# Exidekat/TransformerUpscaler

Measured on AMD Instinct MI355X. Metric: images/sec, FastTransformer 2x 720p->1080p inference, higher is better.
Workload: dtype bf16

## Files before the change

### transformerupscaler_amd/csrc/common.h

```cpp
#pragma once
#include <hip/hip_runtime.h>
#include <stdint.h>
#include <stdlib.h>
#include "tupscale_hip.h"

#ifdef TUP_DIAG
extern "C" {
int tup_debug_tail_stamps(unsigned long long* host_out);
int tup_debug_bs_stamps(unsigned long long* host_out);
int tup_debug_block32_stamps(unsigned long long* host_out);
int tup_debug_conv_stamps(unsigned long long* host_out);
}
#endif

typedef __bf16 bf16_t;
typedef __attribute__((ext_vector_type(8))) __bf16 bf16x8;
typedef __attribute__((ext_vector_type(4))) __bf16 bf16x4;
typedef __attribute__((ext_vector_type(2))) __bf16 bf16x2;
typedef __attribute__((ext_vector_type(4))) short s16x4;
typedef __attribute__((ext_vector_type(4))) float f32x4;
typedef __attribute__((ext_vector_type(4))) uint32_t u32x4;
typedef __attribute__((ext_vector_type(2))) uint32_t u32x2;

#define TUP_DEVICE __device__ __forceinline__

TUP_DEVICE uint32_t lds_addr(const void* p) {
    return (uint32_t)(uintptr_t)(const __attribute__((address_space(3))) char*)(p);
}
TUP_DEVICE bf16x8 lds_read_b128_asm(uint32_t addr) {
    bf16x8 v;
    asm volatile("ds_read_b128 %0, %1" : "=v"(v) : "v"(addr));
    return v;
}
TUP_DEVICE bf16x8 lds_read_b128_asm_off(uint32_t addr, int off) {
    bf16x8 v;
    asm volatile("ds_read_b128 %0, %1 offset:%2" : "=v"(v) : "v"(addr), "i"(off));
    return v;
}
TUP_DEVICE bf16x8 lds_read_b128_asm_off_x64(uint32_t addr, int off) {
    bf16x8 v;
    uint32_t tmp;
    asm volatile("v_xor_b32 %1, 64, %2\n\tds_read_b128 %0, %1 offset:%3" : "=v"(v), "=&v"(tmp) : "v"(addr), "i"(off));
    return v;
}
template <int N> TUP_DEVICE void lds_wait() { asm volatile("s_waitcnt lgkmcnt(%0)" ::"n"(N) : "memory"); }

TUP_DEVICE float bf16_to_f32(bf16_t v) { return static_cast<float>(v); }
TUP_DEVICE bf16_t f32_to_bf16(float v) { return static_cast<bf16_t>(v); }

TUP_DEVICE uint32_t pack_bf16x2(float lo, float hi) {
    bf16x2 p = {static_cast<bf16_t>(lo), static_cast<bf16_t>(hi)};
    return __builtin_bit_cast(uint32_t, p);
}

TUP_DEVICE f32x4 mfma16x16x32(bf16x8 a, bf16x8 b, f32x4 c) {
    return __builtin_amdgcn_mfma_f32_16x16x32_bf16(a, b, c, 0, 0, 0);
}
TUP_DEVICE f32x4 mfma16x16x16(s16x4 a, s16x4 b, f32x4 c) {
    return __builtin_amdgcn_mfma_f32_16x16x16bf16_1k(a, b, c, 0, 0, 0);
}

TUP_DEVICE int swz128(int row, int chunk) { return row * 128 + ((chunk ^ ((row >> 1) & 7)) << 4); }

TUP_DEVICE int lane_id_fresh() {
    int l;
    asm volatile("v_mbcnt_lo_u32_b32 %0, -1, 0\n\tv_mbcnt_hi_u32_b32 %0, -1, %0" : "=v"(l));
    return l;
}
TUP_DEVICE uint32_t opaque_copy(uint32_t u) { asm volatile("" : "+v"(u)); return u; }
TUP_DEVICE float vmax(float a, float b) { float r; asm("v_max_f32 %0, %1, %2" : "=v"(r) : "v"(a), "v"(b)); return r; }
TUP_DEVICE float rows_max(float v) {
    const uint32_t u = __builtin_bit_cast(uint32_t, v);
    const auto r = __builtin_amdgcn_permlane16_swap(u, u, false, false);
    const float m = vmax(__builtin_bit_cast(float, r[0]), __builtin_bit_cast(float, opaque_copy(r[1])));
    const uint32_t w = __builtin_bit_cast(uint32_t, m);
    const auto q = __builtin_amdgcn_permlane32_swap(w, w, false, false);
    return vmax(__builtin_bit_cast(float, q[0]), __builtin_bit_cast(float, opaque_copy(q[1])));
}
TUP_DEVICE float rows_sum(float v) {
    const uint32_t u = __builtin_bit_cast(uint32_t, v);
    const auto r = __builtin_amdgcn_permlane16_swap(u, u, false, false);
    const float m = __builtin_bit_cast(float, r[0]) + __builtin_bit_cast(float, opaque_copy(r[1]));
    const uint32_t w = __builtin_bit_cast(uint32_t, m);
    const auto q = __builtin_amdgcn_permlane32_swap(w, w, false, false);
    return __builtin_bit_cast(float, q[0]) + __builtin_bit_cast(float, opaque_copy(q[1]));
}

typedef __attribute__((ext_vector_type(2))) float f32x2;

TUP_DEVICE f32x2 fast_erf2(f32x2 z) {
    f32x2 zc;
    zc[0] = fminf(fmaxf(z[0], -2.9f), 2.9f);
    zc[1] = fminf(fmaxf(z[1], -2.9f), 2.9f);
    const f32x2 w = zc * zc;
    f32x2 q = w * 1.2033207800518448e-08f + -4.4140491617154536e-07f;
    q = q * w + 6.2528506609435753e-06f;
    q = q * w + -3.6053944566514376e-05f;
    q = q * w + -7.2369640518118916e-05f;
    q = q * w + 0.0026871317284937087f;
    q = q * w + -0.02176163837525465f;
    q = q * w + 0.10692235311582286f;
    q = q * w + -0.37271276562605715f;
    q = q * w + 1.1276929106383919f;
    return zc * q;
}
TUP_DEVICE float fast_erf(float z) { return fast_erf2(f32x2{z, z})[0]; }

template <int N>
TUP_DEVICE void gelu_erf2_batch(f32x2 (&x)[N]) {
    f32x2 xc[N], u[N], q[N];
#pragma unroll
    for (int i = 0; i < N; ++i) {
        xc[i][0] = __builtin_amdgcn_fmed3f(x[i][0], -4.16f, 4.16f);
        xc[i][1] = __builtin_amdgcn_fmed3f(x[i][1], -4.16f, 4.16f);
        u[i] = xc[i] * xc[i];
        q[i] = u[i] * -9.3762207218685175e-10f + 8.1762115989189489e-08f;
    }
    constexpr float C[6] = {-3.0998062963740323e-06f, 6.7728779820009944e-05f, -0.00095683661677124407f, 0.0093223106686782069f,
                            -0.065572048515984249f, 0.39849236879961203f};
#pragma unroll
    for (int k = 0; k < 6; ++k)
#pragma unroll
        for (int i = 0; i < N; ++i) q[i] = q[i] * u[i] + C[k];
#pragma unroll
    for (int i = 0; i < N; ++i) x[i] = x[i] * (xc[i] * q[i] + 0.5f);
}

typedef _Float16 h2 __attribute__((ext_vector_type(2)));
typedef _Float16 h8 __attribute__((ext_vector_type(8)));
template <int N>
TUP_DEVICE void gelu16_batch(h2 (&x)[N]) {
    const h2 one = {(_Float16)1.0f, (_Float16)1.0f};
    h2 xc[N], sv[N], q[N];
#pragma unroll
    for (int i = 0; i < N; ++i) {
        xc[i] = __builtin_elementwise_min(__builtin_elementwise_max(x[i], -one), one);
        sv[i] = __builtin_elementwise_fma(xc[i], xc[i], h2{(_Float16)-0.5f, (_Float16)-0.5f});
        q[i] = __builtin_elementwise_fma(sv[i], h2{(_Float16)1.51615563f, (_Float16)1.51615563f}, h2{(_Float16)-2.11659751f, (_Float16)-2.11659751f});
    }
    constexpr float C[5] = {1.54543088f, -1.13520344f, 0.88632128f, -0.6753973f, 0.70388307f};
#pragma unroll
    for (int k = 0; k < 5; ++k)
#pragma unroll
        for (int i = 0; i < N; ++i) q[i] = __builtin_elementwise_fma(q[i], sv[i], h2{(_Float16)C[k], (_Float16)C[k]});
#pragma unroll
    for (int i = 0; i < N; ++i) x[i] = x[i] * __builtin_elementwise_fma(xc[i], q[i], h2{(_Float16)0.5f, (_Float16)0.5f});
}
template <int TGN>
TUP_DEVICE void gelu16_fragments(const f32x4 (&acc1)[TGN][2], bf16x8 (&hfr)[TGN]) {
    h2 hv[4 * TGN];
#pragma unroll
    for (int tg = 0; tg < TGN; ++tg)
#pragma unroll
        for (int hh = 0; hh < 2; ++hh) {
            hv[tg * 4 + hh * 2 + 0] = __builtin_convertvector(f32x2{acc1[tg][hh][0], acc1[tg][hh][1]}, h2);
            hv[tg * 4 + hh * 2 + 1] = __builtin_convertvector(f32x2{acc1[tg][hh][2], acc1[tg][hh][3]}, h2);
        }
#ifndef TUP_EXP_NOGELU
    gelu16_batch<4 * TGN>(hv);
#endif
#pragma unroll
    for (int tg = 0; tg < TGN; ++tg) {
        u32x4 pk;
#pragma unroll
        for (int q = 0; q < 4; ++q) pk[q] = __builtin_bit_cast(uint32_t, hv[tg * 4 + q]);
        hfr[tg] = __builtin_bit_cast(bf16x8, pk);
    }
}
TUP_DEVICE f32x4 mfma16x16x32_f16(bf16x8 a, bf16x8 b, f32x4 c) {
    return __builtin_amdgcn_mfma_f32_16x16x32_f16(__builtin_bit_cast(h8, a), __builtin_bit_cast(h8, b), c, 0, 0, 0);
}

TUP_DEVICE f32x2 gelu_erf2(f32x2 x) {
    f32x2 v[1] = {x};
    gelu_erf2_batch<1>(v);
    return v[0];
}
TUP_DEVICE float gelu_erf(float x) { return gelu_erf2(f32x2{x, x})[0]; }

TUP_DEVICE float gelu_erf_grad(float x) {
    return 0.5f * (1.0f + fast_erf(x * 0.70710678118654752440f)) + x * 0.39894228040143267794f * __expf(-0.5f * x * x);
}

TUP_DEVICE uint32_t drop_hash(uint32_t seed, uint32_t idx) {
#ifdef TUP_CHEAP_HASH
    return idx * 0x9E3779B1u + seed;
#endif
    uint32_t h = idx * 0x9E3779B1u + seed;
    h ^= h >> 16; h *= 0x85EBCA6Bu; h ^= h >> 13; h *= 0xC2B2AE35u; h ^= h >> 16;
    return h;
}
TUP_DEVICE float drop_scale(uint32_t seed, uint32_t idx, uint32_t thresh, float inv_keep) {
    return drop_hash(seed, idx) >= thresh ? inv_keep : 0.f;
}
TUP_DEVICE float drop_pair_lo(uint32_t h, uint32_t thresh_hi, float inv_keep) { return (h << 16) >= thresh_hi ? inv_keep : 0.f; }
TUP_DEVICE float drop_pair_hi(uint32_t h, uint32_t thresh_hi, float inv_keep) { return h >= thresh_hi ? inv_keep : 0.f; }
TUP_DEVICE float drop_pair(uint32_t seed, uint32_t idx, uint32_t thresh_hi, float inv_keep) {
    const uint32_t h = drop_hash(seed, idx >> 1);
    return ((idx & 1u) ? h : (h << 16)) >= thresh_hi ? inv_keep : 0.f;
}
TUP_DEVICE void drop_pair4(uint32_t seed, uint32_t idx0, uint32_t thresh_hi, float inv_keep, float (&m)[4]) {
    const uint32_t h0 = drop_hash(seed, idx0 >> 1), h1 = drop_hash(seed, (idx0 >> 1) + 1u);
    m[0] = drop_pair_lo(h0, thresh_hi, inv_keep); m[1] = drop_pair_hi(h0, thresh_hi, inv_keep);
    m[2] = drop_pair_lo(h1, thresh_hi, inv_keep); m[3] = drop_pair_hi(h1, thresh_hi, inv_keep);
}
TUP_DEVICE void drop_pair4_rows(uint32_t seed, uint32_t idx0, uint32_t ncols, uint32_t thresh_hi, float inv_keep, float (&m)[4]) {
    const bool odd = (idx0 & 1u) != 0u;
    const uint32_t ia = (idx0 + (odd ? 2u * ncols : 0u)) >> 1;
    const uint32_t ha = drop_hash(seed, ia), hb = drop_hash(seed, ia + (ncols >> 1));
    const uint32_t pa = (uint32_t)__builtin_amdgcn_update_dpp(0, (int)ha, 0xB1, 0xf, 0xf, false);
    const uint32_t pb = (uint32_t)__builtin_amdgcn_update_dpp(0, (int)hb, 0xB1, 0xf, 0xf, false);
    const uint32_t h[4] = {odd ? pa : ha, odd ? pb : hb, odd ? ha : pa, odd ? hb : pb};
#pragma unroll
    for (int e = 0; e < 4; ++e) m[e] = (odd ? h[e] : (h[e] << 16)) >= thresh_hi ? inv_keep : 0.f;
}
inline void drop_pair_params(float p, uint32_t& thresh_hi, float& inv_keep) {
    if (!(p > 0.f)) { thresh_hi = 0u; inv_keep = 1.f; return; }
    long t = (long)((double)p * 65536.0 + 0.5);
    if (t < 1) t = 1;
    if (t > 65535) t = 65535;
    thresh_hi = (uint32_t)t << 16;
    inv_keep = (float)(65536.0 / (65536.0 - (double)t));
}

#define TUP_SET_DYN_LDS(fn, bytes) do { \
        static unsigned long long done_ = 0; int dev_ = 0; \
        hipError_t e_ = hipGetDevice(&dev_); if (e_ != hipSuccess) return (int)e_; \
        if (!((done_ >> (dev_ & 63)) & 1ull)) { \
            e_ = hipFuncSetAttribute((const void*)(fn), hipFuncAttributeMaxDynamicSharedMemorySize, (int)(bytes)); \
            if (e_ != hipSuccess) return (int)e_; \
            done_ |= 1ull << (dev_ & 63); } } while (0)

#ifdef TUP_DIAG
#define TUP_ENV_FLAG(name) (getenv(name) != nullptr)
#define TUP_ENV_INT(name, dflt) (getenv(name) ? atoi(getenv(name)) : (dflt))
#else
#define TUP_ENV_FLAG(name) false
#define TUP_ENV_INT(name, dflt) (dflt)
#endif

#define TUP_CHECK_LAUNCH() do { hipError_t e_ = hipGetLastError(); if (e_ != hipSuccess) return (int)e_; } while (0)

extern "C" int tup_slab_reduce(const float* slab, long long ld, int nslab, float* out, long long n, int accumulate, void* stream);

inline int tup_ln_bwd_det_blocks(int M)
{
    const int groups = (M + 15) / 16;
    const int sweeps = (groups + 255) / 256;
    return (groups + sweeps - 1) / sweeps;
}
```

### transformerupscaler_amd/csrc/conv_pingpong.h

```cpp
#pragma once
#include "common.h"

namespace {

[[maybe_unused]] __device__ __attribute__((aligned(16))) unsigned int tup_zero_line[4] = {0u, 0u, 0u, 0u};
[[maybe_unused]] __device__ __attribute__((aligned(16))) unsigned int tup_store_sink[64 * 8];

#define TUP_ADD_DPP(acc, v, ctrl) asm("v_add_f32_dpp %0, %1, %0 " ctrl " row_mask:0xf bank_mask:0xf bound_ctrl:1" : "+v"(acc) : "v"(v))

TUP_DEVICE uint32_t relu_pack_bf16x2(float lo, float hi) {
    typedef short s16x2 __attribute__((ext_vector_type(2)));
    const bf16x2 v = __builtin_convertvector(f32x2{lo, hi}, bf16x2);
    return __builtin_bit_cast(uint32_t, __builtin_elementwise_max(__builtin_bit_cast(s16x2, v), s16x2{0, 0}));
}

TUP_DEVICE void xcd_band(int total, bool use_bands, int& first, int& stride, int& limit) {
    if ((gridDim.x & 7) == 0 && use_bands) {
        const int band = (total + 7) >> 3, start = (blockIdx.x & 7) * band;
        limit = min(total, start + band);
        first = start + (blockIdx.x >> 3);
        stride = gridDim.x >> 3;
    } else {
        limit = total; first = blockIdx.x; stride = gridDim.x;
    }
}

struct TC { int tx, ty, b; };

struct TileWalk {
    int my_count;
    int nphases;
    TC first;
    int tilesX, tilesY, step_x, step_y, step_b;

    TUP_DEVICE TileWalk(int total_tiles, int tilesX_, int tilesY_, int grp, bool use_bands) : tilesX(tilesX_), tilesY(tilesY_) {
        int first0, per, limit;
        xcd_band(total_tiles, use_bands, first0, per, limit);
        const int first_tile = first0 + grp * per, stride = 2 * per;
        my_count = first_tile < limit ? (limit - first_tile + stride - 1) / stride : 0;
        const int cnt0 = first0 < limit ? (limit - first0 + stride - 1) / stride : 0;
        nphases = 2 * cnt0 + 1;
        first.tx = first_tile % tilesX; const int t = first_tile / tilesX; first.ty = t % tilesY; first.b = t / tilesY;
        step_x = stride % tilesX; step_y = (stride / tilesX) % tilesY; step_b = stride / (tilesX * tilesY);
    }
    TUP_DEVICE void advance(TC& c) const {
        c.tx += step_x;
        if (c.tx >= tilesX) { c.tx -= tilesX; ++c.ty; }
        c.ty += step_y; c.b += step_b;
        if (c.ty >= tilesY) { c.ty -= tilesY; ++c.b; }
    }
};

template <int HALO_H, int HALO_W, int PAD>
struct HaloDma {
    static constexpr int IN_CHUNKS = HALO_H * HALO_W * 8, NPIECE = (IN_CHUNKS + 255) / 256;
    static constexpr bool LAST_PARTIAL = (IN_CHUNKS % 256) != 0;
    int rel[NPIECE];
    int tid, wave;
    bool last_ok;

    TUP_DEVICE HaloDma(int W, int tid_) : tid(tid_), wave(tid_ >> 6), last_ok((NPIECE - 1) * 256 + tid_ < IN_CHUNKS) {
#pragma unroll
        for (int it = 0; it < NPIECE; ++it) {
            const int idx = LAST_PARTIAL ? min(it * 256 + tid, IN_CHUNKS - 1) : it * 256 + tid;
            const int q = idx >> 3, c = (idx & 7) ^ ((q >> 1) & 7);
            const int yy = q / HALO_W, xx = q - yy * HALO_W;
            rel[it] = ((yy - PAD) * W + (xx - PAD)) * 128 + c * 16;
        }
    }
    TUP_DEVICE void prefetch(const bf16_t* x, int b, int ty0, int tx0, int H, int W, char* my_in, const void* zero) const {
        const char* xb = reinterpret_cast<const char*>(x + (size_t)b * H * W * 64);
        if (ty0 >= PAD && ty0 + HALO_H - PAD <= H && tx0 >= PAD && tx0 + HALO_W - PAD <= W) {
            const char* tb = xb + ((size_t)ty0 * W + tx0) * 128;
#pragma unroll
            for (int it = 0; it < NPIECE; ++it) {
                if (LAST_PARTIAL && it == NPIECE - 1 && !last_ok) continue;
                __builtin_amdgcn_global_load_lds((const __attribute__((address_space(1))) void*)(tb + rel[it]),
                                                 (__attribute__((address_space(3))) void*)(my_in + (it * 256 + wave * 64) * 16), 16, 0, 0);
            }
            return;
        }
#pragma unroll 1
        for (int base = 0; base < IN_CHUNKS; base += 256) {
            const int idx = base + tid;
            if (!LAST_PARTIAL || idx < IN_CHUNKS) {
                const int q = idx >> 3, cphys = idx & 7;
                const int c = cphys ^ ((q >> 1) & 7);
                const int yy = q / HALO_W, xx = q - yy * HALO_W;
                const int iy = ty0 - PAD + yy, ix = tx0 - PAD + xx;
                const void* src = (iy >= 0 && iy < H && ix >= 0 && ix < W)
                                      ? (const void*)(xb + ((size_t)(iy * W + ix) * 128 + c * 16)) : zero;
                __builtin_amdgcn_global_load_lds((const __attribute__((address_space(1))) void*)src,
                                                 (__attribute__((address_space(3))) void*)(my_in + (base + wave * 64) * 16), 16, 0, 0);
            }
        }
    }
};

template <int KS, int HALO_W>
TUP_DEVICE void pixel_frag_offsets(uint32_t (&poff)[KS * KS][2], const char* my_in, int wave, int g, int p) {
#pragma unroll
    for (int tap = 0; tap < KS * KS; ++tap)
#pragma unroll
        for (int rw = 0; rw < 2; ++rw)
            poff[tap][rw] = lds_addr(my_in) + (uint32_t)swz128((2 * wave + rw) * HALO_W + p + (tap / KS) * HALO_W + (tap % KS), g);
}
TUP_DEVICE uint32_t weight_frag_base(const char* w_lds, int g, int p) { return lds_addr(w_lds) + (uint32_t)swz128(p, g); }

template <int CT, int NTAPS>
TUP_DEVICE void k_loop(f32x4 (&acc)[4][CT], const uint32_t (&poff)[NTAPS][2], uint32_t wbase0, uint32_t bias_addr) {
    constexpr int WROWS = CT * 16;
    const uint32_t wbase1 = wbase0 ^ 64u;
    const uint32_t wbase0h = wbase0 + 57344u, wbase1h = wbase1 + 57344u;
#pragma unroll
    for (int ct = 0; ct < CT; ++ct) acc[0][ct] = __builtin_bit_cast(f32x4, lds_read_b128_asm(bias_addr + ct * 16));
    lds_wait<0>();
#pragma unroll
    for (int pg = 1; pg < 4; ++pg)
#pragma unroll
        for (int ct = 0; ct < CT; ++ct) acc[pg][ct] = acc[0][ct];
    constexpr int NSTEPS = NTAPS * 2;
    constexpr int PER = 4 + CT;
    constexpr int NM = 4 * CT;
    bf16x8 pf[3][4], wf[3][CT];
    auto load_one = [&](int step, int slot, int j) {
        const int tap = step >> 1;
        if (j < 4) {
            pf[slot][j] = (step & 1) ? lds_read_b128_asm_off_x64(poff[tap][j >> 1], (j & 1) * 2048)
                                     : lds_read_b128_asm_off(poff[tap][j >> 1], (j & 1) * 2048);
        } else {
            const int ct = j - 4;
            const int woff = (tap * WROWS + ct * 16) * 128;
            wf[slot][ct] = woff < 57344 ? lds_read_b128_asm_off((step & 1) ? wbase1 : wbase0, woff)
                                        : lds_read_b128_asm_off((step & 1) ? wbase1h : wbase0h, woff - 57344);
        }
    };
#pragma unroll
    for (int j = 0; j < PER; ++j) load_one(0, 0, j);
#pragma unroll
    for (int j = 0; j < PER; ++j) load_one(1, 1, j);
#pragma unroll
    for (int step = 0; step < NSTEPS; ++step) {
        const int cur = step % 3;
        if (step + 1 < NSTEPS) lds_wait<PER>(); else lds_wait<0>();
        __builtin_amdgcn_sched_barrier(0);
        int rd = 0;
#pragma unroll
        for (int m = 0; m < NM; ++m) {
            if (step + 2 < NSTEPS) {
#pragma unroll
                for (int j = 0; j < PER; ++j)
                    if (j == rd && j * NM < (m + 1) * PER) { load_one(step + 2, (step + 2) % 3, j); ++rd; }
            }
            const int pg = m / CT, ct = m % CT;
            acc[pg][ct] = mfma16x16x32(wf[cur][ct], pf[cur][pg], acc[pg][ct]);
            __builtin_amdgcn_sched_barrier(0);
        }
    }
}

template <int CT, int NTAPS>
TUP_DEVICE void stage_weights(char* w_lds, const bf16_t* wsrc) {
    for (int idx = threadIdx.x; idx < NTAPS * CT * 16 * 8; idx += 512) {
        const int row = idx >> 3, c = idx & 7;
        *reinterpret_cast<u32x4*>(w_lds + swz128(row, c)) = *reinterpret_cast<const u32x4*>(wsrc + (size_t)idx * 8);
    }
}
template <int CT, bool THIN>
TUP_DEVICE void stage_bias(float* bias_lds, const float* bias, int nt, int cout_valid) {
    if (threadIdx.x < 16 * CT) {
        const int gg = threadIdx.x / (4 * CT), ct = (threadIdx.x / 4) % CT, e = threadIdx.x & 3;
        float bval = 0.f;
        if (bias) {
            if constexpr (!THIN) bval = bias[nt * 64 + gg * 16 + ct * 4 + e];
            else { const int co = 16 * ct + 4 * gg + e; bval = co < cout_valid ? bias[co] : 0.f; }
        }
        bias_lds[threadIdx.x] = bval;
    }
}

}
```

### transformerupscaler_amd/csrc/decoder_fused.hip

```cpp
#include "conv_pingpong.h"

namespace {

constexpr int TH = 8, TW = 32, HALO_W = TW + 2, HALO_H = TH + 2, NPIX_HALO = HALO_H * HALO_W;
constexpr int IN_BYTES = NPIX_HALO * 128;
constexpr int WROWS = 64, WSLAB = WROWS * 128;
constexpr size_t DEC_LDS = (size_t)9 * WSLAB + 2 * (size_t)IN_BYTES + 256;
static_assert(DEC_LDS <= 163840, "LDS budget");

__global__ __launch_bounds__(512, 2) void decoder_fused_kernel(
    const bf16_t* __restrict__ x, const bf16_t* __restrict__ wp, const float* __restrict__ bias,
    const bf16_t* __restrict__ wz, float* __restrict__ part, float* __restrict__ seamv, float* __restrict__ cseam,
    int B, int H, int W, int tilesX, int tilesY)
{
    extern __shared__ __attribute__((aligned(16))) char smem[];
    char* w_lds = smem;
    char* in_lds = smem + 9 * WSLAB;

    const int grp = __builtin_amdgcn_readfirstlane((int)(threadIdx.x >> 8));
    const int tid = threadIdx.x & 255, lane = tid & 63, wave = tid >> 6;
    const int g = lane >> 4, p = lane & 15;
    const int total_tiles = tilesX * tilesY * B;
    char* my_in = in_lds + grp * IN_BYTES;

    using Dma = HaloDma<HALO_H, HALO_W, 1>;
    constexpr int NPIECE = Dma::NPIECE;
    const Dma dma(W, tid);
    auto prefetch_tile = [&](const TC& c) { dma.prefetch(x, c.b, c.ty * TH, c.tx * TW, H, W, my_in, tup_zero_line); };

    uint32_t poff[9][2];
    pixel_frag_offsets<3, HALO_W>(poff, my_in, wave, g, p);
    const uint32_t wbase0 = weight_frag_base(w_lds, g, p);

    f32x4 acc[4][4];
    float* bias_lds = reinterpret_cast<float*>(in_lds + 2 * IN_BYTES);
    const uint32_t bias_addr = lds_addr(bias_lds) + (uint32_t)(g * 64);
    bf16x8 zf[3][2];
    const uint32_t wz_voff = (uint32_t)(p * 128 + g * 16);
    auto load_zf = [&]() {
#pragma unroll
        for (int dy = 0; dy < 3; ++dy) {
            const bf16_t* base = wz + dy * 1024;
            asm volatile("global_load_dwordx4 %0, %1, %2" : "=v"(zf[dy][0]) : "v"(wz_voff), "s"(base));
            asm volatile("global_load_dwordx4 %0, %1, %2 offset:64" : "=v"(zf[dy][1]) : "v"(wz_voff), "s"(base));
        }
    };

    auto store_tile = [&](const TC& c) {
        const int b = c.b, y0 = c.ty * TH + 2 * wave, x0 = c.tx * TW;
        const bool edge = c.ty * TH + TH > H || x0 + TW > W;
        f32x4 z[4][3];
#pragma unroll
        for (int pg = 0; pg < 4; ++pg) {
            typedef short s16x2 __attribute__((ext_vector_type(2)));
            uint32_t pk[8];
#pragma unroll
            for (int ct = 0; ct < 4; ++ct) {
                pk[ct * 2 + 0] = pack_bf16x2(acc[pg][ct][0], acc[pg][ct][1]);
                pk[ct * 2 + 1] = pack_bf16x2(acc[pg][ct][2], acc[pg][ct][3]);
            }
#pragma unroll
            for (int q = 0; q < 8; ++q)
                pk[q] = __builtin_bit_cast(uint32_t, __builtin_elementwise_max(__builtin_bit_cast(s16x2, pk[q]), s16x2{0, 0}));
            if (edge) {
                const bool ok = y0 + (pg >> 1) < H && x0 + (pg & 1) * 16 + p < W;
#pragma unroll
                for (int q = 0; q < 8; ++q) pk[q] = ok ? pk[q] : 0u;
            }
            const bf16x8 b0 = __builtin_bit_cast(bf16x8, u32x4{pk[0], pk[1], pk[2], pk[3]});
            const bf16x8 b1 = __builtin_bit_cast(bf16x8, u32x4{pk[4], pk[5], pk[6], pk[7]});
#pragma unroll
            for (int dy = 0; dy < 3; ++dy) {
                z[pg][dy] = mfma16x16x32(zf[dy][0], b0, f32x4{0.f, 0.f, 0.f, 0.f});
                z[pg][dy] = mfma16x16x32(zf[dy][1], b1, z[pg][dy]);
            }
        }
        __builtin_amdgcn_sched_barrier(0);
        asm volatile("s_nop 7\n\ts_nop 7\n\ts_nop 4" ::: "memory");
        __builtin_amdgcn_sched_barrier(0);
        float h[2][2][3];
#pragma unroll
        for (int rw = 0; rw < 2; ++rw)
#pragma unroll
            for (int dy = 0; dy < 3; ++dy) {
                const f32x4 l = z[2 * rw][dy], r = z[2 * rw + 1][dy];
                float v0 = l[1], v1 = r[1];
                TUP_ADD_DPP(v0, l[0], "row_shr:1"); TUP_ADD_DPP(v0, l[2], "row_shl:1"); TUP_ADD_DPP(v0, r[2], "row_shr:15");
                TUP_ADD_DPP(v1, r[0], "row_shr:1"); TUP_ADD_DPP(v1, r[2], "row_shl:1"); TUP_ADD_DPP(v1, l[0], "row_shl:15");
                h[rw][0][dy] = v0; h[rw][1][dy] = v1;
            }
        const bool live = g < 3;
        const int plane = H * W, nrec = 3 * plane * 4;
        const __amdgpu_buffer_rsrc_t rp = __builtin_amdgcn_make_buffer_rsrc(part + (size_t)b * 3 * plane, 0, nrec, 0x00020000);
        const __amdgpu_buffer_rsrc_t rs = __builtin_amdgcn_make_buffer_rsrc(seamv + (size_t)b * 3 * plane, 0, nrec, 0x00020000);
        const int crec = H * tilesX * 128;
        const __amdgpu_buffer_rsrc_t rc = __builtin_amdgcn_make_buffer_rsrc(cseam + (size_t)b * H * tilesX * 32, 0, crec, 0x00020000);
        const int cbase = (g * plane + y0 * W) * 4;
#pragma unroll
        for (int cg = 0; cg < 2; ++cg) {
            const int ox = x0 + cg * 16 + p;
            const bool colok = live && ox < W;
            const int o = cbase + ox * 4, rowb = W * 4;
            const float o0 = h[0][cg][1] + h[1][cg][2], o1 = h[0][cg][0] + h[1][cg][1];
            __builtin_amdgcn_raw_buffer_store_b32(__builtin_bit_cast(uint32_t, o0), rp, colok && y0 < H ? o : nrec, 0, 0);
            __builtin_amdgcn_raw_buffer_store_b32(__builtin_bit_cast(uint32_t, o1), rp, colok && y0 + 1 < H ? o + rowb : nrec, 0, 0);
            __builtin_amdgcn_raw_buffer_store_b32(__builtin_bit_cast(uint32_t, h[0][cg][2]), rs,
                                                  colok && y0 >= 1 && y0 < H ? o - rowb : nrec, 0, 0);
            __builtin_amdgcn_raw_buffer_store_b32(__builtin_bit_cast(uint32_t, h[1][cg][0]), rs,
                                                  colok && y0 + 2 < H ? o + 2 * rowb : nrec, 0, 0);
        }
#pragma unroll
        for (int rw = 0; rw < 2; ++rw) {
            const int y = y0 + rw;
            const bool left = p == 0;
            const f32x4 v = left ? f32x4{z[2 * rw][0][2], z[2 * rw][1][2], z[2 * rw][2][2], 0.f}
                                 : f32x4{z[2 * rw + 1][0][0], z[2 * rw + 1][1][0], z[2 * rw + 1][2][0], 0.f};
            const bool ok = live & (y < H) & (left | ((p == 15) & (x0 + TW <= W)));
            const int off = ((y * tilesX + c.tx) * 2 + (left ? 0 : 1)) * 64 + g * 16;
            __builtin_amdgcn_raw_buffer_store_b128(__builtin_bit_cast(u32x4, v), rc, ok ? off : crec, 0, 0);
        }
    };
    constexpr int NSTORES = 10;

    const TileWalk walk(total_tiles, tilesX, tilesY, grp, true);
    const int my_count = walk.my_count, nphases = walk.nphases;
    const TC c_first = walk.first;

    stage_weights<4, 9>(w_lds, wp);
    stage_bias<4, false>(bias_lds, bias, 0, 64);
    if (grp == 0 && my_count > 0) prefetch_tile(c_first);
    __syncthreads();
    TC c_done = c_first, c_next = c_first;
    if (grp == 0) walk.advance(c_next);

    for (int ph = 0; ph < nphases; ++ph) {
        const int k = ph >> 1;
        if ((ph & 1) == grp) {
            if (k < my_count) k_loop<4, 9>(acc, poff, wbase0, bias_addr);
        } else {
            const int done = grp == 0 ? k : k - 1;
            const int nxt = done + 1;
            const bool store = done >= 0 && done < my_count;
            const bool fetch = nxt < my_count;
            if (store) load_zf();
            if (fetch) prefetch_tile(c_next);
            if (store) {
                if (fetch) asm volatile("s_waitcnt vmcnt(%0)" ::"n"(NPIECE - 1) : "memory");
                else asm volatile("s_waitcnt vmcnt(0)" ::: "memory");
                store_tile(c_done);
                asm volatile("s_waitcnt vmcnt(%0)" ::"n"(NSTORES) : "memory");
            } else {
                asm volatile("s_waitcnt vmcnt(0)" ::: "memory");
            }
            c_done = c_next;
            walk.advance(c_next);
        }
        asm volatile("s_waitcnt lgkmcnt(0)" ::: "memory");
        __builtin_amdgcn_s_barrier();
    }
    asm volatile("s_waitcnt vmcnt(0)" ::: "memory");
}

template <int V>
__global__ __launch_bounds__(256) void decoder_finish_kernel(
    float* __restrict__ res, const float* __restrict__ seamv, const float* __restrict__ cseam, const float* __restrict__ bias,
    int H, int W, int tilesX)
{
    typedef float fv __attribute__((ext_vector_type(V)));
    const int x0 = (blockIdx.x * 256 + threadIdx.x) * V;
    if (x0 >= W) return;
    const int row = blockIdx.y, b = row / H, y = row - b * H;
    const size_t plane = (size_t)H * W;
    const int ys = (y & 1) ? y + 1 : y - 1;
    const bool has_seam = ys >= 0 && ys < H;
    const size_t o0 = (size_t)b * 3 * plane + (size_t)y * W + x0;
#pragma unroll
    for (int c = 0; c < 3; ++c) {
        const size_t o = o0 + c * plane;
        fv v = *reinterpret_cast<const fv*>(res + o);
        const fv sv = has_seam ? *reinterpret_cast<const fv*>(seamv + o) : fv{};
#pragma unroll
        for (int e = 0; e < V; ++e) {
            const int xq = x0 + e;
            float t = bias[c] + v[e];
            if (has_seam) t += sv[e];
            int ctile = -1, side = 0;
            if ((xq & 31) == 31 && xq + 1 < W) { ctile = (xq >> 5) + 1; side = 0; }
            else if ((xq & 31) == 0 && xq > 0) { ctile = (xq >> 5) - 1; side = 1; }
            if (ctile >= 0) {
#pragma unroll
                for (int dy = 0; dy < 3; ++dy) {
                    const int yy = y + dy - 1;
                    if (yy >= 0 && yy < H) t += cseam[((((size_t)b * H + yy) * tilesX + ctile) * 2 + side) * 16 + c * 4 + dy];
                }
            }
            v[e] = t;
        }
        *reinterpret_cast<fv*>(res + o) = v;
    }
}

}

namespace {
int launch_decoder_parts(const void* x, const void* w1, const float* b1, const void* wz, float* part, float* seamv, float* cseam,
                         int B, int H, int W, void* stream)
{
    const int tilesX = (W + TW - 1) / TW, tilesY = (H + TH - 1) / TH;
    const long long nt = (long long)tilesX * tilesY * B;
    if (nt > 0x7fffffffLL || (long long)H * W * 12 > 0x7fffffffLL || (long long)H * tilesX * 128 > 0x7fffffffLL)
        return (int)hipErrorInvalidValue;
    hipStream_t s = reinterpret_cast<hipStream_t>(stream);
    TUP_SET_DYN_LDS(decoder_fused_kernel, DEC_LDS);
    const int grid = (int)(nt < 256 ? nt : 256);
    decoder_fused_kernel<<<dim3(grid), dim3(512), DEC_LDS, s>>>((const bf16_t*)x, (const bf16_t*)w1, b1, (const bf16_t*)wz, part,
                                                                 seamv, cseam, B, H, W, tilesX, tilesY);
    TUP_CHECK_LAUNCH();
    return 0;
}
}

extern "C" int tup_decoder_fused_fwd(const void* x, const void* w1, const float* b1, const void* wz, const float* b2,
                                     float* seamv, float* cseam, float* out, int B, int H, int W, void* stream)
{
    if (B <= 0 || H <= 0 || W <= 0) return 0;
    const int tilesX = (W + TW - 1) / TW;
    if (const int err = launch_decoder_parts(x, w1, b1, wz, out, seamv, cseam, B, H, W, stream)) return err;
    hipStream_t s = reinterpret_cast<hipStream_t>(stream);
    if ((long long)B * H > 0x7fffffffLL) return (int)hipErrorInvalidValue;
    if (W % 4 == 0)
        decoder_finish_kernel<4><<<dim3((unsigned)((W / 4 + 255) / 256), (unsigned)(B * H)), dim3(256), 0, s>>>(out, seamv, cseam, b2, H, W, tilesX);
    else
        decoder_finish_kernel<1><<<dim3((unsigned)((W + 255) / 256), (unsigned)(B * H)), dim3(256), 0, s>>>(out, seamv, cseam, b2, H, W, tilesX);
    TUP_CHECK_LAUNCH();
    return 0;
}

extern "C" int tup_decoder_fused_parts_fwd(const void* x, const void* w1, const float* b1, const void* wz,
                                           float* part, float* seamv, float* cseam, int B, int H, int W, void* stream)
{
    if (B <= 0 || H <= 0 || W <= 0) return 0;
    return launch_decoder_parts(x, w1, b1, wz, part, seamv, cseam, B, H, W, stream);
}
```

Before: 2756.

## Restructure decoder ping-pong handover with wave-owned halo rows and early prologue

Replaces the phase-alternating ping-pong loop in the fused decoder conv with a per-group loop. Each group issues its next tile's bias and first fragment loads before the barrier handover, and waits only for its own halo pieces. The halo DMA is specialised for the 10x34 tile so each wave loads a contiguous set of physically remapped rows, and the LDS fragment offsets follow that row permutation. The aim is to shorten the idle gap at each group handover, at the cost of a more intricate barrier count and a layout tied to one tile shape.

```diff
diff --git a/transformerupscaler_amd/csrc/common.h b/transformerupscaler_amd/csrc/common.h
--- a/transformerupscaler_amd/csrc/common.h
+++ b/transformerupscaler_amd/csrc/common.h
@@ -10,6 +10,7 @@
 int tup_debug_bs_stamps(unsigned long long* host_out);
 int tup_debug_block32_stamps(unsigned long long* host_out);
 int tup_debug_conv_stamps(unsigned long long* host_out);
+int tup_debug_handover_stamps(unsigned long long* host_out);
 }
 #endif
 
diff --git a/transformerupscaler_amd/csrc/conv_pingpong.h b/transformerupscaler_amd/csrc/conv_pingpong.h
--- a/transformerupscaler_amd/csrc/conv_pingpong.h
+++ b/transformerupscaler_amd/csrc/conv_pingpong.h
@@ -1,5 +1,6 @@
 #pragma once
 #include "common.h"
+#include "halo_ownership.h"
 
 namespace {
 
@@ -51,10 +52,12 @@
     }
 };
 
-template <int HALO_H, int HALO_W, int PAD>
+template <int HALO_H, int HALO_W, int PAD, bool OWN = false>
 struct HaloDma {
+    static_assert(!OWN, "wave-owned rows exist for the 10 x 34 image only (the specialisation below)");
     static constexpr int IN_CHUNKS = HALO_H * HALO_W * 8, NPIECE = (IN_CHUNKS + 255) / 256;
     static constexpr bool LAST_PARTIAL = (IN_CHUNKS % 256) != 0;
+    static constexpr int MIN_PIECES = LAST_PARTIAL ? NPIECE - 1 : NPIECE;
     int rel[NPIECE];
     int tid, wave;
     bool last_ok;
@@ -97,33 +100,79 @@
     }
 };
 
-template <int KS, int HALO_W>
+template <>
+struct HaloDma<10, 34, 1, true> {
+    static constexpr int NPIECE = tup_halo_own::NPIECE, MIN_PIECES = NPIECE;
+    int rel[NPIECE];
+    int lane, wave;
+    int own_px, tail_px;
+    bool ok8, ok10;
+
+    TUP_DEVICE int lds_off(int it) const { return tup_halo_own::piece_pixel_at(own_px, tail_px, it) * 128; }
+    TUP_DEVICE HaloDma(int W, int tid_) : lane(tid_ & 63), wave(__builtin_amdgcn_readfirstlane(tid_ >> 6)) {
+        own_px = tup_halo_own::own_base(wave); tail_px = tup_halo_own::tail_base(wave);
+        ok8 = (lane >> 3) < tup_halo_own::piece_npix(wave, 8); ok10 = (lane >> 3) < tup_halo_own::piece_npix(wave, 10);
+#pragma unroll
+        for (int it = 0; it < NPIECE; ++it) {
+            const int q = min((lds_off(it) >> 7) + (lane >> 3), tup_halo_own::NPIX - 1);
+            const int c = (lane & 7) ^ ((q >> 1) & 7);
+            const int prow = q / tup_halo_own::COLS, xx = q - prow * tup_halo_own::COLS, yy = tup_halo_own::logical_row(prow);
+            rel[it] = ((yy - 1) * W + (xx - 1)) * 128 + c * 16;
+        }
+    }
+    TUP_DEVICE void prefetch(const bf16_t* x, int b, int ty0, int tx0, int H, int W, char* my_in, const void* zero) const {
+        const char* xb = reinterpret_cast<const char*>(x + (size_t)b * H * W * 64);
+        if (ty0 >= 1 && ty0 + 9 <= H && tx0 >= 1 && tx0 + 33 <= W) {
+            const char* tb = xb + ((size_t)ty0 * W + tx0) * 128;
+#pragma unroll
+            for (int it = 0; it < NPIECE; ++it) {
+                if ((it == 8 && !ok8) || (it == 10 && !ok10)) continue;
+                __builtin_amdgcn_global_load_lds((const __attribute__((address_space(1))) void*)(tb + rel[it]),
+                                                 (__attribute__((address_space(3))) void*)(my_in + lds_off(it)), 16, 0, 0);
+            }
+            return;
+        }
+#pragma unroll 1
+        for (int it = 0; it < NPIECE; ++it) {
+            if (!((it == 8 && !ok8) || (it == 10 && !ok10))) {
+                const int q = (lds_off(it) >> 7) + (lane >> 3);
+                const int c = (lane & 7) ^ ((q >> 1) & 7);
+                const int prow = q / tup_halo_own::COLS, xx = q - prow * tup_halo_own::COLS, yy = tup_halo_own::logical_row(prow);
+                const int iy = ty0 - 1 + yy, ix = tx0 - 1 + xx;
+                const void* src = (iy >= 0 && iy < H && ix >= 0 && ix < W)
+                                      ? (const void*)(xb + ((size_t)(iy * W + ix) * 128 + c * 16)) : zero;
+                __builtin_amdgcn_global_load_lds((const __attribute__((address_space(1))) void*)src,
+                                                 (__attribute__((address_space(3))) void*)(my_in + lds_off(it)), 16, 0, 0);
+            }
+        }
+    }
+};
+
+template <int KS, int HALO_W, bool OWN = false>
 TUP_DEVICE void pixel_frag_offsets(uint32_t (&poff)[KS * KS][2], const char* my_in, int wave, int g, int p) {
 #pragma unroll
     for (int tap = 0; tap < KS * KS; ++tap)
 #pragma unroll
-        for (int rw = 0; rw < 2; ++rw)
-            poff[tap][rw] = lds_addr(my_in) + (uint32_t)swz128((2 * wave + rw) * HALO_W + p + (tap / KS) * HALO_W + (tap % KS), g);
+        for (int rw = 0; rw < 2; ++rw) {
+            if constexpr (OWN)
+                poff[tap][rw] = lds_addr(my_in) + (uint32_t)swz128(tup_halo_own::phys_row(2 * wave + rw + tap / KS) * HALO_W + p + (tap % KS), g);
+            else
+                poff[tap][rw] = lds_addr(my_in) + (uint32_t)swz128((2 * wave + rw) * HALO_W + p + (tap / KS) * HALO_W + (tap % KS), g);
+        }
 }
 TUP_DEVICE uint32_t weight_frag_base(const char* w_lds, int g, int p) { return lds_addr(w_lds) + (uint32_t)swz128(p, g); }
 
 template <int CT, int NTAPS>
-TUP_DEVICE void k_loop(f32x4 (&acc)[4][CT], const uint32_t (&poff)[NTAPS][2], uint32_t wbase0, uint32_t bias_addr) {
-    constexpr int WROWS = CT * 16;
-    const uint32_t wbase1 = wbase0 ^ 64u;
-    const uint32_t wbase0h = wbase0 + 57344u, wbase1h = wbase1 + 57344u;
-#pragma unroll
-    for (int ct = 0; ct < CT; ++ct) acc[0][ct] = __builtin_bit_cast(f32x4, lds_read_b128_asm(bias_addr + ct * 16));
-    lds_wait<0>();
-#pragma unroll
-    for (int pg = 1; pg < 4; ++pg)
-#pragma unroll
-        for (int ct = 0; ct < CT; ++ct) acc[pg][ct] = acc[0][ct];
-    constexpr int NSTEPS = NTAPS * 2;
-    constexpr int PER = 4 + CT;
-    constexpr int NM = 4 * CT;
+struct KRing {
+    static constexpr int WROWS = CT * 16;
+    static constexpr int NSTEPS = NTAPS * 2;
+    static constexpr int PER = 4 + CT;
+    static constexpr int NM = 4 * CT;
     bf16x8 pf[3][4], wf[3][CT];
-    auto load_one = [&](int step, int slot, int j) {
+
+    TUP_DEVICE void load_one(const uint32_t (&poff)[NTAPS][2], uint32_t wbase0, int step, int slot, int j) {
+        const uint32_t wbase1 = wbase0 ^ 64u;
+        const uint32_t wbase0h = wbase0 + 57344u, wbase1h = wbase1 + 57344u;
         const int tap = step >> 1;
         if (j < 4) {
             pf[slot][j] = (step & 1) ? lds_read_b128_asm_off_x64(poff[tap][j >> 1], (j & 1) * 2048)
@@ -134,29 +183,68 @@
             wf[slot][ct] = woff < 57344 ? lds_read_b128_asm_off((step & 1) ? wbase1 : wbase0, woff)
                                         : lds_read_b128_asm_off((step & 1) ? wbase1h : wbase0h, woff - 57344);
         }
-    };
-#pragma unroll
-    for (int j = 0; j < PER; ++j) load_one(0, 0, j);
-#pragma unroll
-    for (int j = 0; j < PER; ++j) load_one(1, 1, j);
-#pragma unroll
-    for (int step = 0; step < NSTEPS; ++step) {
-        const int cur = step % 3;
-        if (step + 1 < NSTEPS) lds_wait<PER>(); else lds_wait<0>();
-        __builtin_amdgcn_sched_barrier(0);
-        int rd = 0;
-#pragma unroll
-        for (int m = 0; m < NM; ++m) {
-            if (step + 2 < NSTEPS) {
-#pragma unroll
-                for (int j = 0; j < PER; ++j)
-                    if (j == rd && j * NM < (m + 1) * PER) { load_one(step + 2, (step + 2) % 3, j); ++rd; }
-            }
-            const int pg = m / CT, ct = m % CT;
-            acc[pg][ct] = mfma16x16x32(wf[cur][ct], pf[cur][pg], acc[pg][ct]);
+    }
+    TUP_DEVICE void request_first_two(const uint32_t (&poff)[NTAPS][2], uint32_t wbase0) {
+#pragma unroll
+        for (int j = 0; j < PER; ++j) load_one(poff, wbase0, 0, 0, j);
+#pragma unroll
+        for (int j = 0; j < PER; ++j) load_one(poff, wbase0, 1, 1, j);
+    }
+    TUP_DEVICE void steps(f32x4 (&acc)[4][CT], const uint32_t (&poff)[NTAPS][2], uint32_t wbase0) {
+#pragma unroll
+        for (int step = 0; step < NSTEPS; ++step) {
+            const int cur = step % 3;
+            if (step + 1 < NSTEPS) lds_wait<PER>(); else lds_wait<0>();
             __builtin_amdgcn_sched_barrier(0);
-        }
-    }
+            int rd = 0;
+#pragma unroll
+            for (int m = 0; m < NM; ++m) {
+                if (step + 2 < NSTEPS) {
+#pragma unroll
+                    for (int j = 0; j < PER; ++j)
+                        if (j == rd && j * NM < (m + 1) * PER) { load_one(poff, wbase0, step + 2, (step + 2) % 3, j); ++rd; }
+                }
+                const int pg = m / CT, ct = m % CT;
+                acc[pg][ct] = mfma16x16x32(wf[cur][ct], pf[cur][pg], acc[pg][ct]);
+                __builtin_amdgcn_sched_barrier(0);
+            }
+        }
+    }
+};
+
+template <int CT, int NTAPS>
+TUP_DEVICE void k_loop(f32x4 (&acc)[4][CT], const uint32_t (&poff)[NTAPS][2], uint32_t wbase0, uint32_t bias_addr) {
+#pragma unroll
+    for (int ct = 0; ct < CT; ++ct) acc[0][ct] = __builtin_bit_cast(f32x4, lds_read_b128_asm(bias_addr + ct * 16));
+    lds_wait<0>();
+#pragma unroll
+    for (int pg = 1; pg < 4; ++pg)
+#pragma unroll
+        for (int ct = 0; ct < CT; ++ct) acc[pg][ct] = acc[0][ct];
+    KRing<CT, NTAPS> ring;
+    ring.request_first_two(poff, wbase0);
+    ring.steps(acc, poff, wbase0);
+}
+
+template <int CT, int NTAPS>
+TUP_DEVICE void k_prologue(f32x4 (&acc)[4][CT], KRing<CT, NTAPS>& ring, const uint32_t (&poff)[NTAPS][2], uint32_t wbase0, uint32_t bias_addr) {
+#pragma unroll
+    for (int ct = 0; ct < CT; ++ct) acc[0][ct] = __builtin_bit_cast(f32x4, lds_read_b128_asm(bias_addr + ct * 16));
+    ring.request_first_two(poff, wbase0);
+}
+template <int CT>
+TUP_DEVICE void k_bias_wait(f32x4 (&acc)[4][CT]) {
+    static_assert(CT == 4, "the bias wait names four accumulator registers");
+    asm volatile("s_waitcnt lgkmcnt(%4)" : "+v"(acc[0][0]), "+v"(acc[0][1]), "+v"(acc[0][2]), "+v"(acc[0][3]) : "n"(4 + CT) : "memory");
+#pragma unroll
+    for (int pg = 1; pg < 4; ++pg)
+#pragma unroll
+        for (int ct = 0; ct < CT; ++ct) acc[pg][ct] = acc[0][ct];
+}
+template <int CT, int NTAPS>
+TUP_DEVICE void k_main(f32x4 (&acc)[4][CT], KRing<CT, NTAPS>& ring, const uint32_t (&poff)[NTAPS][2], uint32_t wbase0) {
+    k_bias_wait<CT>(acc);
+    ring.steps(acc, poff, wbase0);
 }
 
 template <int CT, int NTAPS>
diff --git a/transformerupscaler_amd/csrc/decoder_fused.hip b/transformerupscaler_amd/csrc/decoder_fused.hip
--- a/transformerupscaler_amd/csrc/decoder_fused.hip
+++ b/transformerupscaler_amd/csrc/decoder_fused.hip
@@ -8,6 +8,15 @@
 constexpr size_t DEC_LDS = (size_t)9 * WSLAB + 2 * (size_t)IN_BYTES + 256;
 static_assert(DEC_LDS <= 163840, "LDS budget");
 
+#ifdef TUP_DIAG
+__device__ unsigned long long tup_handover_stamps[2][4][8][5];
+#define TUP_STAMP(t) asm volatile("s_memtime %0\n\ts_waitcnt lgkmcnt(0)" : "=s"(t)::"memory")
+#define TUP_STAMP_NOWAIT(t) asm volatile("s_memtime %0" : "=s"(t)::"memory")
+#else
+#define TUP_STAMP(t)
+#define TUP_STAMP_NOWAIT(t)
+#endif
+
 __global__ __launch_bounds__(512, 2) void decoder_fused_kernel(
     const bf16_t* __restrict__ x, const bf16_t* __restrict__ wp, const float* __restrict__ bias,
     const bf16_t* __restrict__ wz, float* __restrict__ part, float* __restrict__ seamv, float* __restrict__ cseam,
@@ -23,13 +32,13 @@
     const int total_tiles = tilesX * tilesY * B;
     char* my_in = in_lds + grp * IN_BYTES;
 
-    using Dma = HaloDma<HALO_H, HALO_W, 1>;
-    constexpr int NPIECE = Dma::NPIECE;
+    using Dma = HaloDma<HALO_H, HALO_W, 1, true>;
+    constexpr int MIN_PIECES = Dma::MIN_PIECES;
     const Dma dma(W, tid);
     auto prefetch_tile = [&](const TC& c) { dma.prefetch(x, c.b, c.ty * TH, c.tx * TW, H, W, my_in, tup_zero_line); };
 
     uint32_t poff[9][2];
-    pixel_frag_offsets<3, HALO_W>(poff, my_in, wave, g, p);
+    pixel_frag_offsets<3, HALO_W, true>(poff, my_in, wave, g, p);
     const uint32_t wbase0 = weight_frag_base(w_lds, g, p);
 
     f32x4 acc[4][4];
@@ -130,34 +139,52 @@
     stage_bias<4, false>(bias_lds, bias, 0, 64);
     if (grp == 0 && my_count > 0) prefetch_tile(c_first);
     __syncthreads();
-    TC c_done = c_first, c_next = c_first;
-    if (grp == 0) walk.advance(c_next);
-
-    for (int ph = 0; ph < nphases; ++ph) {
-        const int k = ph >> 1;
-        if ((ph & 1) == grp) {
-            if (k < my_count) k_loop<4, 9>(acc, poff, wbase0, bias_addr);
-        } else {
-            const int done = grp == 0 ? k : k - 1;
-            const int nxt = done + 1;
-            const bool store = done >= 0 && done < my_count;
-            const bool fetch = nxt < my_count;
-            if (store) load_zf();
+    int nbar = 0;
+    if (my_count > 0) {
+        TC c_cur = c_first, c_next = c_first;
+        walk.advance(c_next);
+        KRing<4, 9> ring;
+        if (grp == 1) prefetch_tile(c_cur);
+        asm volatile("s_waitcnt vmcnt(0)" ::: "memory");
+#ifdef TUP_DIAG
+        unsigned long long t_landed = 0, t_rel_a = 0, t_first = 0, t_last = 0, t_rel_b = 0;
+#endif
+        TUP_STAMP(t_landed);
+        k_prologue<4, 9>(acc, ring, poff, wbase0, bias_addr);
+        for (int it = 0;; ++it) {
+            if (grp == 1 || it > 0) { __builtin_amdgcn_s_barrier(); ++nbar; }
+#ifndef TUP_DIAG
+            k_main<4, 9>(acc, ring, poff, wbase0);
+#else
+            TUP_STAMP_NOWAIT(t_rel_a);
+            k_bias_wait<4>(acc);
+            TUP_STAMP_NOWAIT(t_first);
+            ring.steps(acc, poff, wbase0);
+            TUP_STAMP(t_last);
+#endif
+            __builtin_amdgcn_s_barrier(); ++nbar;
+#ifdef TUP_DIAG
+            TUP_STAMP(t_rel_b);
+            if (blockIdx.x == 100 && it < 8 && lane == 0) {
+                unsigned long long* st = tup_handover_stamps[grp][wave][it];
+                st[0] = t_landed; st[1] = t_rel_a; st[2] = t_first; st[3] = t_last; st[4] = t_rel_b;
+            }
+#endif
+            const bool fetch = it + 1 < my_count;
+            load_zf();
             if (fetch) prefetch_tile(c_next);
-            if (store) {
-                if (fetch) asm volatile("s_waitcnt vmcnt(%0)" ::"n"(NPIECE - 1) : "memory");
-                else asm volatile("s_waitcnt vmcnt(0)" ::: "memory");
-                store_tile(c_done);
-                asm volatile("s_waitcnt vmcnt(%0)" ::"n"(NSTORES) : "memory");
-            } else {
-                asm volatile("s_waitcnt vmcnt(0)" ::: "memory");
-            }
-            c_done = c_next;
+            if (fetch) asm volatile("s_waitcnt vmcnt(%0)" ::"n"(MIN_PIECES) : "memory");
+            else asm volatile("s_waitcnt vmcnt(0)" ::: "memory");
+            store_tile(c_cur);
+            if (!fetch) break;
+            asm volatile("s_waitcnt vmcnt(%0)" ::"n"(NSTORES) : "memory");
+            TUP_STAMP(t_landed);
+            k_prologue<4, 9>(acc, ring, poff, wbase0, bias_addr);
+            c_cur = c_next;
             walk.advance(c_next);
         }
-        asm volatile("s_waitcnt lgkmcnt(0)" ::: "memory");
-        __builtin_amdgcn_s_barrier();
     }
+    for (; nbar < nphases; ++nbar) __builtin_amdgcn_s_barrier();
     asm volatile("s_waitcnt vmcnt(0)" ::: "memory");
 }
 
@@ -242,3 +269,10 @@
     if (B <= 0 || H <= 0 || W <= 0) return 0;
     return launch_decoder_parts(x, w1, b1, wz, part, seamv, cseam, B, H, W, stream);
 }
+
+#ifdef TUP_DIAG
+extern "C" int tup_debug_handover_stamps(unsigned long long* host_out)
+{
+    return (int)hipMemcpyFromSymbol(host_out, HIP_SYMBOL(tup_handover_stamps), sizeof(unsigned long long) * 2 * 4 * 8 * 5);
+}
+#endif
diff --git a/transformerupscaler_amd/csrc/halo_ownership.h b/transformerupscaler_amd/csrc/halo_ownership.h
--- /dev/null
+++ b/transformerupscaler_amd/csrc/halo_ownership.h
@@ -0,0 +1,16 @@
+#pragma once
+
+namespace tup_halo_own {
+
+constexpr int ROWS = 10, COLS = 34, NPIX = ROWS * COLS, NWAVES = 4, NPIECE = 11;
+
+constexpr int phys_row(int row) { return row < 2 ? row : row < 8 ? row + 2 : row - 6; }
+constexpr int logical_row(int prow) { return prow < 2 ? prow : prow < 4 ? prow + 6 : prow - 2; }
+
+constexpr int own_base(int wave) { return wave == 0 ? 0 : wave == 1 ? 116 : wave == 2 ? 204 : 272; }
+constexpr int tail_base(int wave) { return wave == 0 ? 72 : wave == 1 ? 188 : wave == 2 ? 88 : 102; }
+constexpr int piece_pixel_at(int own, int tail, int it) { return it < 9 ? own + 8 * it : tail + 8 * (it - 9); }
+constexpr int piece_pixel(int wave, int it) { return piece_pixel_at(own_base(wave), tail_base(wave), it); }
+constexpr int piece_npix(int wave, int it) { return wave < 2 ? 8 : it == 8 ? 4 : it == 10 ? 6 : 8; }
+
+}
```

Result: no change. 2752 (-0.1%).
